# yukiteruono/pbsim3

Measured on AMD Instinct MI355X. Metric: simulated bases/sec, higher is better.
Workload: dtype u8

## Files before the change

pbsim3_amd/csrc/deflate.hip:

```cpp
#include <hip/hip_runtime.h>
#include <stdint.h>
#include <stdlib.h>

#include "kernels.h"

namespace pbsim {

namespace {

constexpr int kChunk = DF_CHUNK;
constexpr int kThreads = 256;
constexpr int kSeg = kChunk / kThreads;
constexpr int kSegDw = kSeg / 4;
constexpr int kInDw = kChunk / 4 + kChunk / 128;
constexpr int kOutBytes = 33024;
constexpr int kOutDw = kOutBytes / 4;
constexpr int kSyms = 288;
constexpr uint32_t kPoly = 0xEDB88320u;
constexpr int kHeadBits = 18 * 8;
constexpr int kPrefixBits = 3 + 5 + 5 + 4 + 19 * 3;

constexpr int kClLenTab[19] = {3, 5, 4, 4, 4, 5, 5, 5, 5, 5, 5, 5, 4, 5, 5, 5, 5, 3, 3};
constexpr int kClOrderTab[19] = {16, 17, 18, 0, 8, 7, 9, 6, 10, 5, 11, 4, 12, 3, 13, 2, 14, 1, 15};
constexpr uint64_t pack_cl_len() {
  uint64_t v = 0;
  for (int s = 0; s < 19; ++s) v |= (uint64_t)kClLenTab[s] << (3 * s);
  return v;
}
constexpr uint64_t kClLenPacked = pack_cl_len();
__device__ __forceinline__ uint32_t cl_len(uint32_t s) { return (uint32_t)(kClLenPacked >> (3 * s)) & 7u; }
constexpr unsigned __int128 pack_prefix() {
  unsigned __int128 v = 1u | (2u << 1) | ((unsigned __int128)15 << 13);
  for (int i = 0; i < 19; ++i) v |= (unsigned __int128)kClLenTab[kClOrderTab[i]] << (17 + 3 * i);
  return v;
}
constexpr uint64_t kPrefixLo = (uint64_t)pack_prefix();
constexpr uint32_t kPrefixHi = (uint32_t)(pack_prefix() >> 64);

__device__ __forceinline__ uint32_t rev_bits(uint32_t code, uint32_t len) { return __brev(code) >> (32 - len); }

__device__ __forceinline__ uint32_t cl_code(uint32_t s) {
  uint32_t c, l = cl_len(s);
  if (l == 3) c = s == 0 ? 0 : s - 16;
  else if (l == 4) c = s == 12 ? 9 : 4 + s;
  else c = s == 1 ? 20 : s <= 11 ? 16 + s : 15 + s;
  return rev_bits(c, l);
}

__device__ __forceinline__ uint32_t gf2_mul(uint32_t a, uint32_t b) {
  uint32_t p = 0;
#pragma unroll
  for (int i = 0; i < 32; ++i) {
    p ^= b & (0u - ((a >> (31 - i)) & 1u));
    b = (b >> 1) ^ (kPoly & (0u - (b & 1u)));
  }
  return p;
}

struct BitWriter {
  uint32_t *out;
  uint32_t word, nb;
  uint64_t acc;
  __device__ __forceinline__ void init(uint32_t *o, uint32_t bitpos) {
    out = o;
    word = bitpos >> 5;
    nb = bitpos & 31;
    acc = 0;
  }
  __device__ __forceinline__ void put(uint32_t v, uint32_t k) {
    acc |= (uint64_t)v << nb;
    nb += k;
    if (nb >= 32) {
      atomicOr(&out[word++], (uint32_t)acc);
      acc >>= 32;
      nb -= 32;
    }
  }
  __device__ __forceinline__ void put64(uint64_t v, uint32_t k) {
    if (k > 32) {
      put((uint32_t)v, 32);
      put((uint32_t)(v >> 32), k - 32);
    } else {
      put((uint32_t)v, k);
    }
  }
  __device__ __forceinline__ void flush() {
    if (nb) atomicOr(&out[word], (uint32_t)acc);
  }
};

__device__ __forceinline__ void length_symbol(uint32_t L, uint32_t *sym, uint32_t *eb, uint32_t *ev) {
  const uint32_t v = L - 3;
  if (v < 8) {
    *sym = 257 + v;
    *eb = 0;
    *ev = 0;
  } else if (L == 258) {
    *sym = 285;
    *eb = 0;
    *ev = 0;
  } else {
    const uint32_t e = (31 - __clz(v)) - 2;
    *sym = 261 + 4 * e + ((v >> e) & 3);
    *eb = e;
    *ev = v & ((1u << e) - 1);
  }
}

__device__ __forceinline__ uint32_t block_scan_excl(uint32_t v, uint32_t *s_wave, uint32_t *total) {
  const int lane = threadIdx.x & 63, wave = threadIdx.x >> 6;
  uint32_t inc = v;
#pragma unroll
  for (int d = 1; d < 64; d <<= 1) {
    const uint32_t o = __shfl_up(inc, d, 64);
    if (lane >= d) inc += o;
  }
  __syncthreads();
  if (lane == 63) s_wave[wave] = inc;
  __syncthreads();
  uint32_t base = 0, tot = 0;
#pragma unroll
  for (int w = 0; w < kThreads / 64; ++w) {
    const uint32_t x = s_wave[w];
    if (w < wave) base += x;
    tot += x;
  }
  *total = tot;
  return base + inc - v;
}

struct Mask128 {
  uint64_t lo, hi;
};
__device__ __forceinline__ Mask128 m_and(Mask128 a, Mask128 b) { return {a.lo & b.lo, a.hi & b.hi}; }
__device__ __forceinline__ Mask128 m_or(Mask128 a, Mask128 b) { return {a.lo | b.lo, a.hi | b.hi}; }
__device__ __forceinline__ Mask128 m_not(Mask128 a) { return {~a.lo, ~a.hi}; }
template <int K>
__device__ __forceinline__ Mask128 m_shl(Mask128 a) { return {a.lo << K, (a.hi << K) | (a.lo >> (64 - K))}; }
template <int K>
__device__ __forceinline__ Mask128 m_shr(Mask128 a) { return {(a.lo >> K) | (a.hi << (64 - K)), a.hi >> K}; }
__device__ __forceinline__ uint32_t m_nibble(Mask128 a, int j) {
  return (uint32_t)((j < 16 ? a.lo >> (4 * j) : a.hi >> (4 * j - 64)) & 15u);
}
__device__ __forceinline__ int m_first(Mask128 a) { return a.lo ? __builtin_ctzll(a.lo) : 64 + __builtin_ctzll(a.hi); }
__device__ __forceinline__ Mask128 m_clear(Mask128 a, int pos) {
  if (pos < 64) a.lo &= ~(1ull << pos);
  else a.hi &= ~(1ull << (pos - 64));
  return a;
}
__device__ __forceinline__ int m_run(Mask128 m, int pos) {
  uint64_t lo, hi;
  if (pos == 0) {
    lo = m.lo;
    hi = m.hi;
  } else if (pos < 64) {
    lo = (m.lo >> pos) | (m.hi << (64 - pos));
    hi = m.hi >> pos;
  } else {
    lo = m.hi >> (pos - 64);
    hi = 0;
  }
  if (~lo) return __builtin_ctzll(~lo);
  return ~hi ? 64 + __builtin_ctzll(~hi) : 128;
}

struct SegTokens {
  Mask128 lit;
  Mask128 start;
  Mask128 cover;
};

__device__ __forceinline__ SegTokens seg_tokens(const uint32_t (&seg)[kSegDw], int seg_n, uint32_t prev_dword,
                                                bool chunk_start) {
  uint64_t e[2] = {0, 0};
  uint32_t pw = prev_dword;
#pragma unroll
  for (int j = 0; j < kSegDw; ++j) {
    const uint32_t w = seg[j];
    const uint32_t d = w ^ ((w << 8) | (pw >> 24));
    const uint32_t z = ~(((d & 0x7F7F7F7Fu) + 0x7F7F7F7Fu) | d | 0x7F7F7F7Fu);
    const uint32_t nib = (((z >> 7) * 0x00204081u) >> 21) & 15u;
    e[j >> 4] |= (uint64_t)nib << (4 * (j & 15));
    pw = w;
  }
  Mask128 valid;
  valid.lo = seg_n >= 64 ? ~0ull : (1ull << seg_n) - 1;
  valid.hi = seg_n >= 128 ? ~0ull : seg_n > 64 ? (1ull << (seg_n - 64)) - 1 : 0ull;
  Mask128 eq = {e[0] & valid.lo, e[1] & valid.hi};
  if (chunk_start) eq.lo &= ~1ull;
  const Mask128 r3 = m_and(eq, m_and(m_shr<1>(eq), m_shr<2>(eq)));
  SegTokens t;
  t.cover = m_or(r3, m_or(m_shl<1>(r3), m_shl<2>(r3)));
  t.start = m_and(t.cover, m_not(m_shl<1>(t.cover)));
  t.lit = m_and(valid, m_not(t.cover));
  return t;
}

constexpr int kSampleChunks = DF_SAMPLE_CHUNKS;
constexpr int kHdrDw = DF_TABLE_HDR_DW;

struct DfTable {
  uint32_t code[kSyms];
  uint32_t hdr_end_bits;
  uint32_t pad[3];
  uint32_t hdr[kHdrDw];
};
static_assert(sizeof(DfTable) <= DF_TABLE_BYTES, "DF_TABLE_BYTES too small");

__device__ __forceinline__ void load_chunk(const uint8_t *__restrict__ text, int64_t n_bytes, int64_t chunk, uint32_t *s_in,
                                           uint32_t (&seg)[kSegDw], int *n_out, int *seg_n_out, uint32_t *prev_dw) {
  const int tid = threadIdx.x;
  const int64_t base = chunk * (int64_t)kChunk;
  const int n = (int)((n_bytes - base) < (int64_t)kChunk ? (n_bytes - base) : (int64_t)kChunk);
  const uint4 *src4 = reinterpret_cast<const uint4 *>(text + base);
  for (int q = tid; q < kChunk / 16; q += kThreads) {
    uint4 v = make_uint4(0, 0, 0, 0);
    if (q * 16 < n) v = src4[q];
    const int d = q * 4;
    uint32_t *dst = &s_in[d + (d >> 5)];
    dst[0] = v.x;
    dst[1] = v.y;
    dst[2] = v.z;
    dst[3] = v.w;
  }
  __syncthreads();
  const int beg = tid * kSeg;
  *n_out = n;
  *seg_n_out = n - beg < 0 ? 0 : (n - beg < kSeg ? n - beg : kSeg);
#pragma unroll
  for (int j = 0; j < kSegDw; ++j) seg[j] = s_in[tid * (kSegDw + 1) + j];
  *prev_dw = tid ? s_in[tid * (kSegDw + 1) - 2] : 0u;
  __syncthreads();
}

__global__ __launch_bounds__(kThreads) void k_deflate_hist(const uint8_t *__restrict__ text, int64_t n_bytes,
                                                            uint32_t *__restrict__ hist) {
  __shared__ uint32_t s_in[kInDw];
  __shared__ uint32_t s_hist[3 * kSyms + 64];
  const int tid = threadIdx.x, lane = tid & 63;
  for (int i = tid; i < 3 * kSyms + 64; i += kThreads) s_hist[i] = 0;
  uint32_t seg[kSegDw], prev_dw;
  int n, seg_n;
  load_chunk(text, n_bytes, blockIdx.x, s_in, seg, &n, &seg_n, &prev_dw);
  const SegTokens tk = seg_tokens(seg, seg_n, prev_dw, tid == 0);
  const uint32_t copy = (uint32_t)(lane % 3) * kSyms, dummy = 3 * kSyms + lane;
#pragma unroll
  for (int j = 0; j < kSegDw; ++j) {
    const uint32_t nl = m_nibble(tk.lit, j);
    if (nl == 0) continue;
    const uint32_t w = seg[j];
#pragma unroll
    for (int k = 0; k < 4; ++k) atomicAdd(&s_hist[((nl >> k) & 1u) ? copy + ((w >> (8 * k)) & 255u) : dummy], 1u);
  }
  Mask128 st = tk.start;
  while (st.lo | st.hi) {
    const int pos = m_first(st);
    st = m_clear(st, pos);
    uint32_t sy, eb, ev;
    length_symbol((uint32_t)m_run(tk.cover, pos), &sy, &eb, &ev);
    atomicAdd(&s_hist[copy + sy], 1u);
  }
  __syncthreads();
  for (int i = tid; i < 286; i += kThreads) {
    const uint32_t f = s_hist[i] + s_hist[kSyms + i] + s_hist[2 * kSyms + i] + (i == 256 ? 1u : 0u);
    if (f) atomicAdd(&hist[i], f);
  }
}

__global__ __launch_bounds__(kThreads) void k_deflate_build(const uint32_t *__restrict__ hist, DfTable *__restrict__ tbl) {
  __shared__ uint32_t s_freq[kSyms], s_sfreq[kSyms], s_w[kSyms], s_code[kSyms];
  __shared__ uint16_t s_sorted[kSyms], s_par[kSyms], s_leafpar[kSyms], s_dep[kSyms];
  __shared__ uint8_t s_len[kSyms];
  __shared__ uint32_t s_cnt[16], s_first[16];
  __shared__ uint32_t s_img[4 + kHdrDw];
  const int tid = threadIdx.x;
  constexpr int m = 286;
  for (int i = tid; i < kSyms; i += kThreads) {
    s_freq[i] = i < m ? hist[i] + 1u : 0u;
    s_code[i] = 0;
    s_len[i] = 0;
  }
  for (int i = tid; i < 4 + kHdrDw; i += kThreads) s_img[i] = 0;
  if (tid < 16) s_cnt[tid] = 0;
  __syncthreads();
  for (int i = tid; i < m; i += kThreads) {
    const uint32_t fi = s_freq[i];
    uint32_t rank = 0;
    for (int u = 0; u < m; ++u) {
      const uint32_t g = s_freq[u];
      rank += (g < fi) | ((g == fi) & (u < i));
    }
    s_sorted[rank] = (uint16_t)i;
    s_sfreq[rank] = fi;
  }
  __syncthreads();
  if (tid == 0) {
    int leaf = 0, root = 0;
    for (int nxt = 0; nxt < m - 1; ++nxt) {
      uint32_t tot = 0;
      for (int k = 0; k < 2; ++k) {
        const bool take_leaf = leaf < m && (root >= nxt || s_sfreq[leaf] <= s_w[root]);
        if (take_leaf) {
          tot += s_sfreq[leaf];
          s_leafpar[leaf] = (uint16_t)nxt;
          ++leaf;
        } else {
          tot += s_w[root];
          s_par[root] = (uint16_t)nxt;
          ++root;
        }
      }
      s_w[nxt] = tot;
    }
    s_dep[m - 2] = 0;
    for (int i = m - 3; i >= 0; --i) s_dep[i] = s_dep[s_par[i]] + 1;
    for (int i = 0; i < m; ++i) {
      int d = s_dep[s_leafpar[i]] + 1;
      if (d > 15) d = 15;
      s_cnt[d] += 1;
    }
    uint32_t total = 0;
    for (int l = 1; l <= 15; ++l) total += s_cnt[l] << (15 - l);
    while (total > (1u << 15)) {
      s_cnt[15] -= 1;
      for (int l = 14; l >= 1; --l)
        if (s_cnt[l]) {
// ... 52 lines not shown
  for (int i = tid; i < kHdrDw; i += kThreads) tbl->hdr[i] = s_img[4 + i];
}

struct DfCtl {
  uint32_t ticket;
  uint32_t error;
  int64_t total;
};
static_assert(sizeof(DfCtl) == DF_CTL_BYTES, "DF_CTL_BYTES");

constexpr uint64_t kStSize = 1ull << 32, kStPrefix = 2ull << 32;
__device__ __forceinline__ uint64_t st_word(uint32_t epoch, uint64_t flag, uint32_t v) { return ((uint64_t)epoch << 34) | flag | v; }

__device__ __forceinline__ uint32_t look_back(const uint64_t *status, int64_t c, uint32_t epoch, int lane, uint32_t *error) {
  uint32_t sum = 0;
  int64_t hi = c - 1;
  for (uint32_t spins = 0;; spins++) {
    if (spins > (1u << 24)) {
      if (lane == 0) atomicOr(error, 1u);
      return sum;
    }
    const int64_t i = hi - lane;
    uint64_t w = 0;
    if (i >= 0) w = __hip_atomic_load(&status[i], __ATOMIC_RELAXED, __HIP_MEMORY_SCOPE_AGENT);
    const bool mine = i >= 0 && (uint32_t)(w >> 34) == epoch && ((w >> 32) & 3u) != 0;
    const uint64_t ready = __ballot(mine || i < 0);
    const uint64_t pref = __ballot(mine && ((w >> 32) & 3u) == 2u);
    const int k = ~ready ? __builtin_ctzll(~ready) : 64;
    const uint64_t usable = k >= 64 ? ~0ull : ((1ull << k) - 1);
    const uint64_t stop = pref & usable;
    if (stop) {
      const int e = __builtin_ctzll(stop);
      uint32_t v = (lane <= e && i >= 0) ? (uint32_t)w : 0u;
#pragma unroll
      for (int d = 32; d >= 1; d >>= 1) v += __shfl_xor(v, d, 64);
      return sum + v;
    }
    if (k == 0) {
      __builtin_amdgcn_s_sleep(2);
      continue;
    }
    uint32_t v = (lane < k && i >= 0) ? (uint32_t)w : 0u;
#pragma unroll
    for (int d = 32; d >= 1; d >>= 1) v += __shfl_xor(v, d, 64);
    sum += v;
    hi -= k;
    if (hi < 0) return sum;
  }
}

typedef uint32_t u32x4 __attribute__((ext_vector_type(4)));
__device__ __forceinline__ void store_member(uint8_t *dst, const uint32_t *s_img, uint32_t bytes, int tid) {
  const uint32_t head = min((uint32_t)((16u - ((uintptr_t)dst & 15u)) & 15u), bytes);
  const uint8_t *s8 = reinterpret_cast<const uint8_t *>(s_img);
  if ((uint32_t)tid < head) dst[tid] = s8[tid];
  const uint32_t nvec = (bytes - head) >> 4;
  const uint32_t sh = head & 3u, dw0 = head >> 2;
  u32x4 *d4 = reinterpret_cast<u32x4 *>(dst + head);
  for (uint32_t v = tid; v < nvec; v += kThreads) {
    const uint32_t *p = s_img + dw0 + 4u * v;
    const uint32_t a = p[0], b = p[1], c = p[2], d = p[3], e = p[4];
    u32x4 o;
    o.x = __builtin_amdgcn_alignbyte(b, a, sh);
    o.y = __builtin_amdgcn_alignbyte(c, b, sh);
    o.z = __builtin_amdgcn_alignbyte(d, c, sh);
    o.w = __builtin_amdgcn_alignbyte(e, d, sh);
    __builtin_nontemporal_store(o, &d4[v]);
  }
  const uint32_t done = head + 16u * nvec;
  if ((uint32_t)tid < bytes - done) dst[done + tid] = s8[done + tid];
}

__global__ __launch_bounds__(kThreads) void k_deflate_chunks(const uint8_t *__restrict__ text, int64_t n_bytes,
                                                              uint8_t *__restrict__ dense, uint64_t *__restrict__ status,
                                                              DfCtl *__restrict__ ctl, uint32_t epoch,
                                                              const uint32_t *__restrict__ crc_table,
                                                              const uint32_t *__restrict__ pow128, uint32_t x8rem,
                                                              const DfTable *__restrict__ tbl,
                                                              unsigned long long *__restrict__ prof) {
  __shared__ uint32_t s_in[kInDw];
  static_assert(kOutDw <= kInDw, "the output image must fit the input image");
  uint32_t *const s_out = s_in;
  __shared__ uint32_t s_code[kSyms];
  uint32_t *const s_crc = s_in;
  __shared__ uint32_t s_wave[kThreads / 64];
  __shared__ uint32_t s_misc[4];

  const int tid = threadIdx.x, lane = tid & 63;
  unsigned long long t_prev = prof ? wall_clock64() : 0;
  int phase = 0;
  auto mark = [&]() {
    if (prof && tid == 0) {
      const unsigned long long t = wall_clock64();
      atomicAdd(&prof[phase], t - t_prev);
      t_prev = t;
    }
    ++phase;
  };
  for (int i = tid; i < kSyms; i += kThreads) s_code[i] = i < 286 ? tbl->code[i] : 0u;
  if (tid < 4) s_misc[tid] = tid == 0 ? atomicAdd(&ctl->ticket, 1u) : 0u;
  __syncthreads();
  const int64_t chunk = s_misc[0];
  const int64_t n_chunks = (n_bytes + kChunk - 1) / kChunk;
  uint32_t seg[kSegDw], prev_dw;
  int n, seg_n;
  load_chunk(text, n_bytes, chunk, s_in, seg, &n, &seg_n, &prev_dw);
  const int beg = tid * kSeg;
  mark();
  for (int i = tid; i < kInDw; i += kThreads) s_in[i] = (i < 1024) ? crc_table[i] : 0u;
  __syncthreads();
  const SegTokens tk = seg_tokens(seg, seg_n, prev_dw, tid == 0);

  uint32_t tok_bits = 0;
  {
    uint32_t c = tid == 0 ? 0xFFFFFFFFu : 0u;
    const int full = seg_n >> 2;
#pragma unroll
    for (int j = 0; j < kSegDw; ++j) {
      if (j < full) {
        const uint32_t x = c ^ seg[j];
        c = s_crc[768 + (x & 255u)] ^ s_crc[512 + ((x >> 8) & 255u)] ^ s_crc[256 + ((x >> 16) & 255u)] ^ s_crc[x >> 24];
      } else if (j == full) {
        for (int k = 0; k < (seg_n & 3); ++k) c = s_crc[(c ^ (seg[j] >> (8 * k))) & 255u] ^ (c >> 8);
      }
    }
    const int q = n >> 7, r = n & 127;
    if (seg_n == kSeg && tid < q) {
      c = gf2_mul(c, pow128[q - tid - 1]);
      if (r) c = gf2_mul(c, x8rem);
    }
    if (seg_n == 0) c = 0;
#pragma unroll
    for (int d = 32; d >= 1; d >>= 1) c ^= __shfl_xor(c, d, 64);
    if (lane == 0) atomicXor(&s_misc[3], c);
  }
  mark();
  {
#pragma unroll
    for (int j = 0; j < kSegDw; ++j) {
      const uint32_t nl = m_nibble(tk.lit, j);
      if (nl == 0) continue;
      const uint32_t w = seg[j];
#pragma unroll
      for (int k = 0; k < 4; ++k)
        tok_bits += s_code[((nl >> k) & 1u) ? (w >> (8 * k)) & 255u : 287u] >> 16;
    }
    Mask128 st = tk.start;
    while (st.lo | st.hi) {
      const int pos = m_first(st);
      st = m_clear(st, pos);
      uint32_t sy, eb, ev;
      length_symbol((uint32_t)m_run(tk.cover, pos), &sy, &eb, &ev);
      tok_bits += (s_code[sy] >> 16) + eb + 1;
    }
  }
  uint32_t tok_total;
  const uint32_t tok_off = block_scan_excl(tok_bits, s_wave, &tok_total);
  const uint32_t hdr_end = tbl->hdr_end_bits;
  const uint32_t eob_len = s_code[256] >> 16;
  const uint32_t payload_bits = hdr_end - kHeadBits + tok_total + eob_len;
  const uint32_t payload_bytes = (payload_bits + 7) >> 3;
  const bool huff = (18 + payload_bytes + 8 <= (uint32_t)kOutBytes) && (payload_bytes < (uint32_t)n + 5);
  const uint32_t crc = s_misc[3] ^ 0xFFFFFFFFu;
  const uint32_t member = huff ? 18 + payload_bytes + 8 : 18 + 5 + (uint32_t)n + 8;
  if (tid == 0)
    __hip_atomic_store(&status[chunk], st_word(epoch, chunk == 0 ? kStPrefix : kStSize, member), __ATOMIC_RELAXED, __HIP_MEMORY_SCOPE_AGENT);
  mark();

  if (huff) {
    __syncthreads();
    for (int i = tid; i < 1024; i += kThreads) s_in[i] = 0;
    __syncthreads();
    if (tid < kHdrDw) s_out[4 + tid] = tbl->hdr[tid];
    if (tid == 0) {
      s_out[0] = 0x04088b1fu;
      s_out[1] = 0;
      s_out[2] = 0x0006ff00u;
      s_out[3] = 0x00024342u;
    }
    __syncthreads();
    if (tid == 0) atomicOr(&s_out[4], member - 1);
    mark();
    {
      BitWriter bw;
      bw.init(s_out, hdr_end + tok_off);
#pragma unroll
      for (int j = 0; j < kSegDw; ++j) {
        const uint32_t nl = m_nibble(tk.lit, j), ns = m_nibble(tk.start, j);
        if ((nl | ns) == 0) continue;
        const uint32_t w = seg[j];
        uint32_t c[4];
#pragma unroll
        for (int k = 0; k < 4; ++k) c[k] = s_code[((nl >> k) & 1u) ? (w >> (8 * k)) & 255u : 287u];
        uint32_t mv = 0, ml = 0, ks = 4;
        if (ns) {
          ks = (uint32_t)__builtin_ctz(ns);
          uint32_t sy, eb, ev;
          length_symbol((uint32_t)m_run(tk.cover, 4 * j + (int)ks), &sy, &eb, &ev);
          const uint32_t cm = s_code[sy];
          mv = (cm & 0xFFFFu) | (ev << (cm >> 16));
          ml = (cm >> 16) + eb + 1;
        }
        bw.put(ks == 0 ? mv : 0u, ks == 0 ? ml : 0u);
        {
          const uint32_t l0 = c[0] >> 16;
          bw.put((c[0] & 0xFFFFu) | ((c[1] & 0xFFFFu) << l0), l0 + (c[1] >> 16));
        }
        const bool mid = ks == 1 || ks == 2;
        bw.put(mid ? mv : 0u, mid ? ml : 0u);
        {
          const uint32_t l2 = c[2] >> 16;
          bw.put((c[2] & 0xFFFFu) | ((c[3] & 0xFFFFu) << l2), l2 + (c[3] >> 16));
        }
        bw.put(ks == 3 ? mv : 0u, ks == 3 ? ml : 0u);
      }
      bw.flush();
    }
    mark();
    if (tid == 0) {
      BitWriter bw;
      bw.init(s_out, hdr_end + tok_total);
      bw.put(s_code[256] & 0xFFFFu, eob_len);
      bw.flush();
      bw.init(s_out, (18 + payload_bytes) * 8);
      bw.put(crc, 32);
      bw.put((uint32_t)n, 32);
      bw.flush();
    }
    if (tid < 64 && chunk > 0) {
      const uint32_t excl = look_back(status, chunk, epoch, tid, &ctl->error);
      if (tid == 0) {
        s_misc[1] = excl;
        __hip_atomic_store(&status[chunk], st_word(epoch, kStPrefix, excl + member), __ATOMIC_RELAXED, __HIP_MEMORY_SCOPE_AGENT);
      }
    }
    __syncthreads();
    mark();
    const uint32_t off = s_misc[1];
    store_member(dense + off, s_out, member, tid);
    if (tid == 0 && chunk == n_chunks - 1) ctl->total = (int64_t)off + member;
    mark();
  } else {
    if (tid < 64 && chunk > 0) {
      const uint32_t excl = look_back(status, chunk, epoch, tid, &ctl->error);
      if (tid == 0) {
        s_misc[1] = excl;
        __hip_atomic_store(&status[chunk], st_word(epoch, kStPrefix, excl + member), __ATOMIC_RELAXED, __HIP_MEMORY_SCOPE_AGENT);
      }
    }
    __syncthreads();
    uint8_t *slot = dense + s_misc[1];
    if (tid == 0 && chunk == n_chunks - 1) ctl->total = (int64_t)s_misc[1] + member;
    if (tid == 0) {
      const uint8_t head[23] = {0x1f, 0x8b, 8,   4,   0,   0,
                                0,    0,    0,   0xff, 6,  0,
                                'B',  'C',  2,   0,   (uint8_t)((member - 1) & 255), (uint8_t)((member - 1) >> 8),
                                1,    (uint8_t)(n & 255), (uint8_t)(n >> 8), (uint8_t)(~n & 255), (uint8_t)((~n >> 8) & 255)};
      for (int i = 0; i < 23; ++i) slot[i] = head[i];
      uint8_t *t = slot + 23 + n;
      for (int i = 0; i < 4; ++i) t[i] = (uint8_t)(crc >> (8 * i));
      for (int i = 0; i < 4; ++i) t[4 + i] = (uint8_t)((uint32_t)n >> (8 * i));
    }
#pragma unroll
    for (int j = 0; j < kSegDw; ++j)
#pragma unroll
      for (int k = 0; k < 4; ++k)
        if (4 * j + k < seg_n) slot[23 + beg + 4 * j + k] = (uint8_t)(seg[j] >> (8 * k));
  }
}

uint32_t host_gf2_mul(uint32_t a, uint32_t b) {
  uint32_t p = 0;
  for (int i = 0; i < 32; ++i) {
    if (a & (0x80000000u >> i)) p ^= b;
    b = (b >> 1) ^ ((b & 1u) ? kPoly : 0u);
  }
  return p;
}

uint32_t host_xpow8(uint64_t nbytes) {
  uint32_t r = 0x80000000u, b = 0x00800000u;
  while (nbytes) {
    if (nbytes & 1) r = host_gf2_mul(r, b);
    b = host_gf2_mul(b, b);
    nbytes >>= 1;
  }
  return r;
}

}

void deflate_host_tables(uint32_t *crc_table, uint32_t *pow128) {
  for (uint32_t i = 0; i < 256; ++i) {
    uint32_t c = i;
    for (int k = 0; k < 8; ++k) c = (c >> 1) ^ ((c & 1u) ? kPoly : 0u);
    crc_table[i] = c;
  }
  for (int t = 1; t < 4; ++t)
    for (uint32_t i = 0; i < 256; ++i) {
      const uint32_t c = crc_table[(t - 1) * 256 + i];
      crc_table[t * 256 + i] = (c >> 8) ^ crc_table[c & 255u];
    }
  const uint32_t step = host_xpow8(128);
  uint32_t v = 0x80000000u;
  for (int k = 0; k < 256; ++k) {
    pow128[k] = v;
    v = host_gf2_mul(v, step);
  }
}

void launch_deflate_table(const uint8_t *text, int64_t n_bytes, uint32_t *hist, void *table, hipStream_t s) {
  if (n_bytes <= 0) return;
  const int64_t nch = (n_bytes + DF_CHUNK - 1) / DF_CHUNK;
  const int64_t ns = nch < kSampleChunks ? nch : kSampleChunks;
  const int64_t sample_bytes = ns * (int64_t)DF_CHUNK < n_bytes ? ns * (int64_t)DF_CHUNK : n_bytes;
  (void)hipMemsetAsync(hist, 0, 288 * sizeof(uint32_t), s);
  hipLaunchKernelGGL(k_deflate_hist, dim3((unsigned)ns), dim3(kThreads), 0, s, text, sample_bytes, hist);
  hipLaunchKernelGGL(k_deflate_build, dim3(1), dim3(kThreads), 0, s, (const uint32_t *)hist, reinterpret_cast<DfTable *>(table));
}

void launch_deflate(const uint8_t *text, int64_t n_bytes, uint64_t *status, void *ctl, uint32_t epoch, uint8_t *dense,
                    const uint32_t *d_crc_table, const uint32_t *d_pow128, const void *table, hipStream_t s,
                    unsigned long long *d_prof, hipEvent_t ev_begin, hipEvent_t ev_chunks_done) {
  if (n_bytes <= 0) return;
  const int64_t nch = (n_bytes + DF_CHUNK - 1) / DF_CHUNK;
  const uint32_t x8rem = host_xpow8((uint64_t)(n_bytes % DF_CHUNK) & 127u);
  (void)hipMemsetAsync(ctl, 0, DF_CTL_BYTES, s);
  if (ev_begin) (void)hipEventRecord(ev_begin, s);
  hipLaunchKernelGGL(k_deflate_chunks, dim3((unsigned)nch), dim3(kThreads), 0, s, text, n_bytes, dense, status,
                     reinterpret_cast<DfCtl *>(ctl), epoch & 0x3fffffffu, d_crc_table, d_pow128, x8rem,
                     reinterpret_cast<const DfTable *>(table), d_prof);
  if (ev_chunks_done) (void)hipEventRecord(ev_chunks_done, s);
}

}
```

pbsim3_amd/csrc/deflate_host.cpp:

```cpp
#include <hip/hip_runtime.h>
#include <limits.h>
#include <math.h>
#include <stdio.h>
#include <stdlib.h>
#include <string.h>

#include <algorithm>
#include <chrono>
#include <functional>
#include <memory>
#include <string>
#include <thread>
#include <vector>

#include "ctx.h"
#include "engine_internal.h"
#include "unit_io.h"

extern "C" {

extern "C++" {
namespace {

int ensure_deflate_tables(pbsim_ctx *c) {
// ... 129 lines not shown
  bool used[kDfBuffers] = {false};
  int64_t *h_total = reinterpret_cast<int64_t *>(sl.h_df_total.p);
  auto launch = [&](int64_t j) -> int {
    return df_launch_piece(c, sl, g, d_text, n, j, used[(int)(j % nbuf)], place == nullptr, d_prof);
  };
  for (int64_t j = sl.pre_count; j < std::min<int64_t>(ahead, n_pieces); j++)
    if (!launch(j)) return PBSIM_FAILED;
  const char *prev_ptr = nullptr;
  int64_t prev_bytes = 0;
  int prev_buf = 0;
  for (int64_t k = 0; k < n_pieces; k++) {
    const int b = (int)(k % nbuf);
    const double t0 = now();
    HIP_OK(hipEventSynchronize(sl.ev_df[b]));
    t_kernel += now() - t0;
    const int64_t total = h_total[2 * b + 1];
    if ((uint64_t)h_total[2 * b] >> 32) return fail("deflate: a workgroup's look-back gave up waiting for its predecessors");
    out_bytes += total;
    {
      float ms = 0;
      if (hipEventElapsedTime(&ms, sl.ev_k0[b], sl.ev_k1[b]) == hipSuccess) {
        std::lock_guard<std::mutex> lk(c->prof_mu);
        c->prof_deflate_ms += ms;
        c->prof_deflate_launches++;
        c->prof_deflate_in += g.len(k, n);
        c->prof_deflate_out += total;
      }
    }
    char *dst = place ? (*place)(total) : (char *)sl.h_df_out[b].p;
    if (!dst) return fail("deflate: no room for a compressed piece");
    HIP_OK(hipStreamWaitEvent(sl.copy_stream, sl.ev_df[b], 0));
    if (trace) {
      hipEvent_t e0 = nullptr, e1 = nullptr;
      HIP_OK(hipEventCreate(&e0));
      HIP_OK(hipEventCreate(&e1));
      tev.emplace_back(e0, e1);
      HIP_OK(hipEventRecord(e0, sl.copy_stream));
    }
    HIP_OK(hipMemcpyAsync(dst, sl.d_df_dense[b].p, (size_t)total, hipMemcpyDeviceToHost, sl.copy_stream));
    if (trace) HIP_OK(hipEventRecord(tev.back().second, sl.copy_stream));
    HIP_OK(hipEventRecord(sl.ev_cp[b], sl.copy_stream));
    used[b] = true;
    if (prev_bytes) {
      const double t1 = now();
      HIP_OK(hipEventSynchronize(sl.ev_cp[prev_buf]));
      const double t2 = now();
      if (!consume(prev_ptr, prev_bytes)) return PBSIM_FAILED;
      t_copy += t2 - t1;
      t_consume += now() - t2;
    }
    prev_ptr = dst;
    prev_bytes = total;
    prev_buf = b;
    if (k + ahead < n_pieces && !launch(k + ahead)) return PBSIM_FAILED;
  }
  if (prev_bytes) {
    const double t1 = now();
    HIP_OK(hipEventSynchronize(sl.ev_cp[prev_buf]));
    const double t2 = now();
    if (!consume(prev_ptr, prev_bytes)) return PBSIM_FAILED;
    t_copy += t2 - t1;
    t_consume += now() - t2;
  }
  if (trace) {
    double t_link = 0, t_span = 0;
    float ms = 0;
    for (auto &e : tev) {
      if (hipEventElapsedTime(&ms, e.first, e.second) == hipSuccess) t_link += ms;
    }
    if (!tev.empty() && hipEventElapsedTime(&ms, tev.front().first, tev.back().second) == hipSuccess) t_span = ms;
    for (auto &e : tev) {
      (void)hipEventDestroy(e.first);
      (void)hipEventDestroy(e.second);
    }
    fprintf(stderr,
            "[deflate] %.1f MB -> %.1f MB in %.1f ms: waited %.1f ms for kernels, %.1f ms for copies, %.1f ms in the consumer; copies: "
            "%.1f ms on the engine within a span of %.1f ms (%.1f GB/s while copying)\n",
            n / 1e6, out_bytes / 1e6, now() - t_begin, t_kernel, t_copy, t_consume, t_link, t_span, t_link > 0 ? out_bytes / t_link / 1e6 : 0.0);
  }
  if (d_prof) {
    unsigned long long t[16];
    HIP_OK(hipMemcpy(t, d_prof, 128, hipMemcpyDeviceToHost));
    const double nch = (double)((n + DF_CHUNK - 1) / DF_CHUNK);
    static const char *names[7] = {"stage", "crc", "sizes+scan", "header", "tokens", "trailer", "store"};
    fprintf(stderr, "[deflate prof] %.0f chunks; us per chunk (lane 0):", nch);
    for (int i = 0; i < 7; ++i) fprintf(stderr, " %s %.1f", names[i], t[i] / nch / 100);
    fprintf(stderr, "\n");
  }
  return PBSIM_SUCCEEDED;
}

int deflate_to_host(pbsim_ctx *c, DfLane &sl, const uint8_t *d_text, int64_t n, char *host_dst, int64_t cap,
                    int64_t *out_bytes) {
  int64_t written = 0;
  const int ok = deflate_stream(c, sl, d_text, n, [&](const char *z, int64_t k) {
    if (written + k > cap) return fail("deflate: output buffer too small");
    memcpy(host_dst + written, z, (size_t)k);
    written += k;
    return PBSIM_SUCCEEDED;
  });
  *out_bytes = written;
  return ok;
}

}
}

extern "C++" int pbsim::deflate_pieces(pbsim_ctx *c, DfLane &lane, const uint8_t *d_text, int64_t n,
                                       const std::function<int(const char *, int64_t)> &consume,
                                       const std::function<char *(int64_t)> *place) {
  return deflate_stream(c, lane, d_text, n, consume, place);
}
extern "C++" int pbsim::ensure_deflate_ready(pbsim_ctx *c) {
  for (auto &lane : c->df_streams)
    for (hipStream_t &st : lane)
      if (!st) HIP_OK(hipStreamCreateWithFlags(&st, hipStreamNonBlocking));
  return ensure_deflate_tables(c);
}
extern "C++" int pbsim::ensure_crc_tables(pbsim_ctx *c) { return ensure_deflate_tables(c); }
extern "C++" int pbsim::deflate_prelaunch(pbsim_ctx *c, Slot &sl, bool want_read, bool want_maf) {
  const pbsim_batch_info &bi = sl.b_info;
  if (want_read && bi.read_text_bytes > 0 && !df_begin(c, sl.df[0], sl.d_read_text.as<uint8_t>(), bi.read_text_bytes, true, sl.stream))
    return PBSIM_FAILED;
  if (want_maf && bi.maf_text_bytes > 0 && !df_begin(c, sl.df[1], sl.d_maf_text.as<uint8_t>(), bi.maf_text_bytes, true, sl.stream))
    return PBSIM_FAILED;
  return PBSIM_SUCCEEDED;
}

int pbsim_set_deflate(pbsim_ctx *c, int on) {
  if (!c) return fail("bad argument");
  c->deflate = on & 3;
  c->deflate_parallel = (on & 4) != 0;
  return PBSIM_SUCCEEDED;
}

int64_t pbsim_deflate_bound(int64_t n) {
  if (n <= 0) return 0;
  return n + ((n + DF_CHUNK - 1) / DF_CHUNK) * 31;
}

int pbsim_batch_fetch_deflated(pbsim_ctx *c, char *read_gz, int64_t read_cap, char *maf_gz, int64_t maf_cap,
                               int64_t *read_gz_bytes, int64_t *maf_gz_bytes) {
  if (!c || !c->s().b_finalized) return fail("pbsim_batch_fetch_deflated: no finalized batch");
  NEED_DEVICE(c);
  HIP_OK(hipSetDevice(c->device));
  int64_t nr = 0, nm = 0;
  if (read_gz && !deflate_to_host(c, c->s().df[0], c->s().d_read_text.as<uint8_t>(), c->s().b_info.read_text_bytes, read_gz,
                                  read_cap, &nr))
    return PBSIM_FAILED;
  if (maf_gz && !deflate_to_host(c, c->s().df[0], c->s().d_maf_text.as<uint8_t>(), c->s().b_info.maf_text_bytes, maf_gz,
                                 maf_cap, &nm))
    return PBSIM_FAILED;
  if (read_gz_bytes) *read_gz_bytes = nr;
  if (maf_gz_bytes) *maf_gz_bytes = nm;
  return PBSIM_SUCCEEDED;
}

int pbsim_deflate_buffer(pbsim_ctx *c, const void *src, int64_t n, void *dst, int64_t cap, int64_t *out_bytes) {
  if (!c || !out_bytes || n < 0 || (n > 0 && (!src || !dst))) return fail("pbsim_deflate_buffer: bad argument");
  NEED_DEVICE(c);
  HIP_OK(hipSetDevice(c->device));
  *out_bytes = 0;
  if (n == 0) return PBSIM_SUCCEEDED;
  Slot &sl = c->slots[0];
  DevBuf d_in;
  HIP_OK(d_in.ensure((size_t)n + 16));
  HIP_OK(hipMemcpyAsync(d_in.p, src, (size_t)n, hipMemcpyHostToDevice, sl.stream));
  HIP_OK(hipStreamSynchronize(sl.stream));
  return deflate_to_host(c, sl.df[0], d_in.as<uint8_t>(), n, (char *)dst, cap, out_bytes);
// ... 68 lines not shown
```

Before: 56.38 billion.

## Make deflate kernel persistent with prefetch of next chunk and resident CRC table

Turns k_deflate_chunks into a persistent kernel: the grid is capped at the number of resident workgroups, and each workgroup loops over chunks taken from the ticket counter. The next chunk's global load is issued before the current member is stored, so the fetch overlaps the store. The CRC table, header dwords and code table are now loaded once per workgroup into a dedicated shared array instead of once per chunk. The zeroing of the output image is limited to the member size, and the bit writer uses branchless puts. The cost is 4 KB more LDS per workgroup, which may lower occupancy, and more register pressure from keeping the prefetched quads live.

Measured after the change: 56.38 billion (median of 3 runs). No clear change (+0.0%).

```diff
diff --git a/pbsim3_amd/csrc/deflate.hip b/pbsim3_amd/csrc/deflate.hip
--- a/pbsim3_amd/csrc/deflate.hip
+++ b/pbsim3_amd/csrc/deflate.hip
@@ -1,6 +1,9 @@
 #include <hip/hip_runtime.h>
 #include <stdint.h>
 #include <stdlib.h>
+
+#include <algorithm>
+#include <atomic>
 
 #include "kernels.h"
 
@@ -75,6 +78,15 @@
       acc >>= 32;
       nb -= 32;
     }
+  }
+  __device__ __forceinline__ void put_always(uint32_t v, uint32_t k) {
+    acc |= (uint64_t)v << nb;
+    nb += k;
+    atomicOr(&out[word], (uint32_t)acc);
+    const bool full = nb >= 32;
+    word += full ? 1u : 0u;
+    acc = full ? acc >> 32 : acc;
+    nb &= 31u;
   }
   __device__ __forceinline__ void put64(uint64_t v, uint32_t k) {
     if (k > 32) {
@@ -107,8 +119,8 @@
   }
 }
 
-__device__ __forceinline__ uint32_t block_scan_excl(uint32_t v, uint32_t *s_wave, uint32_t *total) {
-  const int lane = threadIdx.x & 63, wave = threadIdx.x >> 6;
+__device__ __forceinline__ uint32_t block_scan_excl(uint32_t v, uint32_t *s_wave, uint32_t *total, int tid) {
+  const int lane = tid & 63, wave = tid >> 6;
   uint32_t inc = v;
 #pragma unroll
   for (int d = 1; d < 64; d <<= 1) {
@@ -207,30 +219,40 @@
 };
 static_assert(sizeof(DfTable) <= DF_TABLE_BYTES, "DF_TABLE_BYTES too small");
 
-__device__ __forceinline__ void load_chunk(const uint8_t *__restrict__ text, int64_t n_bytes, int64_t chunk, uint32_t *s_in,
-                                           uint32_t (&seg)[kSegDw], int *n_out, int *seg_n_out, uint32_t *prev_dw) {
-  const int tid = threadIdx.x;
-  const int64_t base = chunk * (int64_t)kChunk;
-  const int n = (int)((n_bytes - base) < (int64_t)kChunk ? (n_bytes - base) : (int64_t)kChunk);
-  const uint4 *src4 = reinterpret_cast<const uint4 *>(text + base);
-  for (int q = tid; q < kChunk / 16; q += kThreads) {
-    uint4 v = make_uint4(0, 0, 0, 0);
-    if (q * 16 < n) v = src4[q];
-    const int d = q * 4;
+constexpr int kQuads = kChunk / 16 / kThreads;
+__device__ __forceinline__ int chunk_bytes(int64_t n_bytes, int64_t chunk) {
+  const int64_t left = n_bytes - chunk * (int64_t)kChunk;
+  return (int)(left < 0 ? 0 : left < (int64_t)kChunk ? left : (int64_t)kChunk);
+}
+__device__ __forceinline__ void chunk_fetch(const uint8_t *__restrict__ text, int64_t n_bytes, int64_t chunk, uint4 (&quad)[kQuads], int tid) {
+  const int n = chunk_bytes(n_bytes, chunk);
+  const uint4 *src4 = reinterpret_cast<const uint4 *>(text + chunk * (int64_t)kChunk);
+#pragma unroll
+  for (int i = 0; i < kQuads; ++i) {
+    const int q = tid + i * kThreads;
+    quad[i] = make_uint4(0, 0, 0, 0);
+    if (q * 16 < n) quad[i] = src4[q];
+  }
+}
+__device__ __forceinline__ void chunk_land(const uint4 (&quad)[kQuads], int64_t n_bytes, int64_t chunk, uint32_t *s_in,
+                                           uint32_t (&seg)[kSegDw], int *n_out, int *seg_n_out, uint32_t *prev_dw, int tid) {
+#pragma unroll
+  for (int i = 0; i < kQuads; ++i) {
+    const int d = (tid + i * kThreads) * 4;
     uint32_t *dst = &s_in[d + (d >> 5)];
-    dst[0] = v.x;
-    dst[1] = v.y;
-    dst[2] = v.z;
-    dst[3] = v.w;
-  }
-  __syncthreads();
+    dst[0] = quad[i].x;
+    dst[1] = quad[i].y;
+    dst[2] = quad[i].z;
+    dst[3] = quad[i].w;
+  }
+  __syncthreads();
+  const int n = chunk_bytes(n_bytes, chunk);
   const int beg = tid * kSeg;
   *n_out = n;
   *seg_n_out = n - beg < 0 ? 0 : (n - beg < kSeg ? n - beg : kSeg);
 #pragma unroll
   for (int j = 0; j < kSegDw; ++j) seg[j] = s_in[tid * (kSegDw + 1) + j];
   *prev_dw = tid ? s_in[tid * (kSegDw + 1) - 2] : 0u;
-  __syncthreads();
 }
 
 __global__ __launch_bounds__(kThreads) void k_deflate_hist(const uint8_t *__restrict__ text, int64_t n_bytes,
@@ -241,7 +263,9 @@
   for (int i = tid; i < 3 * kSyms + 64; i += kThreads) s_hist[i] = 0;
   uint32_t seg[kSegDw], prev_dw;
   int n, seg_n;
-  load_chunk(text, n_bytes, blockIdx.x, s_in, seg, &n, &seg_n, &prev_dw);
+  uint4 quad[kQuads];
+  chunk_fetch(text, n_bytes, blockIdx.x, quad, tid);
+  chunk_land(quad, n_bytes, blockIdx.x, s_in, seg, &n, &seg_n, &prev_dw, tid);
   const SegTokens tk = seg_tokens(seg, seg_n, prev_dw, tid == 0);
   const uint32_t copy = (uint32_t)(lane % 3) * kSyms, dummy = 3 * kSyms + lane;
 #pragma unroll
@@ -460,190 +484,205 @@
   static_assert(kOutDw <= kInDw, "the output image must fit the input image");
   uint32_t *const s_out = s_in;
   __shared__ uint32_t s_code[kSyms];
-  uint32_t *const s_crc = s_in;
+  __shared__ uint32_t s_crc[1024];
   __shared__ uint32_t s_wave[kThreads / 64];
   __shared__ uint32_t s_misc[4];
 
-  const int tid = threadIdx.x, lane = tid & 63;
+  const int tid0 = threadIdx.x;
   unsigned long long t_prev = prof ? wall_clock64() : 0;
-  int phase = 0;
+  int phase = 7;
   auto mark = [&]() {
-    if (prof && tid == 0) {
+    if (prof && tid0 == 0) {
       const unsigned long long t = wall_clock64();
       atomicAdd(&prof[phase], t - t_prev);
       t_prev = t;
     }
     ++phase;
   };
-  for (int i = tid; i < kSyms; i += kThreads) s_code[i] = i < 286 ? tbl->code[i] : 0u;
-  if (tid < 4) s_misc[tid] = tid == 0 ? atomicAdd(&ctl->ticket, 1u) : 0u;
-  __syncthreads();
-  const int64_t chunk = s_misc[0];
   const int64_t n_chunks = (n_bytes + kChunk - 1) / kChunk;
-  uint32_t seg[kSegDw], prev_dw;
-  int n, seg_n;
-  load_chunk(text, n_bytes, chunk, s_in, seg, &n, &seg_n, &prev_dw);
-  const int beg = tid * kSeg;
+  for (int i = tid0; i < kSyms; i += kThreads) s_code[i] = i < 286 ? tbl->code[i] : 0u;
+  for (int i = tid0; i < 1024; i += kThreads) s_crc[i] = crc_table[i];
+  static_assert(kHdrDw <= kThreads, "one header dword per thread");
+  const uint32_t my_hdr = tid0 < kHdrDw ? tbl->hdr[tid0] : 0u;
+  const uint32_t hdr_end = tbl->hdr_end_bits;
+  if (tid0 < 4) s_misc[tid0] = tid0 == 0 ? atomicAdd(&ctl->ticket, 1u) : 0u;
+  __syncthreads();
+  int64_t chunk = s_misc[0];
+  const uint32_t eob = s_code[256], eob_len = eob >> 16;
+  uint4 quad[kQuads];
+  chunk_fetch(text, n_bytes, chunk, quad, tid0);
   mark();
-  for (int i = tid; i < kInDw; i += kThreads) s_in[i] = (i < 1024) ? crc_table[i] : 0u;
-  __syncthreads();
-  const SegTokens tk = seg_tokens(seg, seg_n, prev_dw, tid == 0);
-
-  uint32_t tok_bits = 0;
-  {
-    uint32_t c = tid == 0 ? 0xFFFFFFFFu : 0u;
-    const int full = seg_n >> 2;
-#pragma unroll
-    for (int j = 0; j < kSegDw; ++j) {
-      if (j < full) {
-        const uint32_t x = c ^ seg[j];
-        c = s_crc[768 + (x & 255u)] ^ s_crc[512 + ((x >> 8) & 255u)] ^ s_crc[256 + ((x >> 16) & 255u)] ^ s_crc[x >> 24];
-      } else if (j == full) {
-        for (int k = 0; k < (seg_n & 3); ++k) c = s_crc[(c ^ (seg[j] >> (8 * k))) & 255u] ^ (c >> 8);
-      }
-    }
-    const int q = n >> 7, r = n & 127;
-    if (seg_n == kSeg && tid < q) {
-      c = gf2_mul(c, pow128[q - tid - 1]);
-      if (r) c = gf2_mul(c, x8rem);
-    }
-    if (seg_n == 0) c = 0;
-#pragma unroll
-    for (int d = 32; d >= 1; d >>= 1) c ^= __shfl_xor(c, d, 64);
-    if (lane == 0) atomicXor(&s_misc[3], c);
-  }
-  mark();
-  {
-#pragma unroll
-    for (int j = 0; j < kSegDw; ++j) {
-      const uint32_t nl = m_nibble(tk.lit, j);
-      if (nl == 0) continue;
-      const uint32_t w = seg[j];
-#pragma unroll
-      for (int k = 0; k < 4; ++k)
-        tok_bits += s_code[((nl >> k) & 1u) ? (w >> (8 * k)) & 255u : 287u] >> 16;
-    }
-    Mask128 st = tk.start;
-    while (st.lo | st.hi) {
-      const int pos = m_first(st);
-      st = m_clear(st, pos);
-      uint32_t sy, eb, ev;
-      length_symbol((uint32_t)m_run(tk.cover, pos), &sy, &eb, &ev);
-      tok_bits += (s_code[sy] >> 16) + eb + 1;
-    }
-  }
-  uint32_t tok_total;
-  const uint32_t tok_off = block_scan_excl(tok_bits, s_wave, &tok_total);
-  const uint32_t hdr_end = tbl->hdr_end_bits;
-  const uint32_t eob_len = s_code[256] >> 16;
-  const uint32_t payload_bits = hdr_end - kHeadBits + tok_total + eob_len;
-  const uint32_t payload_bytes = (payload_bits + 7) >> 3;
-  const bool huff = (18 + payload_bytes + 8 <= (uint32_t)kOutBytes) && (payload_bytes < (uint32_t)n + 5);
-  const uint32_t crc = s_misc[3] ^ 0xFFFFFFFFu;
-  const uint32_t member = huff ? 18 + payload_bytes + 8 : 18 + 5 + (uint32_t)n + 8;
-  if (tid == 0)
-    __hip_atomic_store(&status[chunk], st_word(epoch, chunk == 0 ? kStPrefix : kStSize, member), __ATOMIC_RELAXED, __HIP_MEMORY_SCOPE_AGENT);
-  mark();
-
-  if (huff) {
-    __syncthreads();
-    for (int i = tid; i < 1024; i += kThreads) s_in[i] = 0;
-    __syncthreads();
-    if (tid < kHdrDw) s_out[4 + tid] = tbl->hdr[tid];
-    if (tid == 0) {
-      s_out[0] = 0x04088b1fu;
-      s_out[1] = 0;
-      s_out[2] = 0x0006ff00u;
-      s_out[3] = 0x00024342u;
-    }
-    __syncthreads();
-    if (tid == 0) atomicOr(&s_out[4], member - 1);
+
+  while (chunk < n_chunks) {
+    phase = 0;
+    int tid = tid0;
+    __asm__ volatile("" : "+v"(tid));
+    __asm__ volatile("" : "+s"(x8rem));
+    const int lane = tid & 63;
+    uint32_t seg[kSegDw], prev_dw;
+    int n, seg_n;
+    chunk_land(quad, n_bytes, chunk, s_in, seg, &n, &seg_n, &prev_dw, tid);
+    const int beg = tid * kSeg;
+    mark();
+    SegTokens tk = seg_tokens(seg, seg_n, prev_dw, tid == 0);
+
+    uint32_t tok_bits = 0;
+    {
+      uint32_t c = tid == 0 ? 0xFFFFFFFFu : 0u;
+      const int full = seg_n >> 2;
+#pragma unroll
+      for (int j = 0; j < kSegDw; ++j) {
+        if (j < full) {
+          const uint32_t x = c ^ seg[j];
+          c = s_crc[768 + (x & 255u)] ^ s_crc[512 + ((x >> 8) & 255u)] ^ s_crc[256 + ((x >> 16) & 255u)] ^ s_crc[x >> 24];
+        } else if (j == full) {
+          for (int k = 0; k < (seg_n & 3); ++k) c = s_crc[(c ^ (seg[j] >> (8 * k))) & 255u] ^ (c >> 8);
+        }
+      }
+      const int q = n >> 7, r = n & 127;
+      if (seg_n == kSeg && tid < q) {
+        c = gf2_mul(c, pow128[q - tid - 1]);
+        if (r) c = gf2_mul(c, x8rem);
+      }
+      if (seg_n == 0) c = 0;
+#pragma unroll
+      for (int d = 32; d >= 1; d >>= 1) c ^= __shfl_xor(c, d, 64);
+      if (lane == 0) atomicXor(&s_misc[3], c);
+    }
     mark();
     {
-      BitWriter bw;
-      bw.init(s_out, hdr_end + tok_off);
 #pragma unroll
       for (int j = 0; j < kSegDw; ++j) {
-        const uint32_t nl = m_nibble(tk.lit, j), ns = m_nibble(tk.start, j);
-        if ((nl | ns) == 0) continue;
+        const uint32_t nl = m_nibble(tk.lit, j);
+        if (nl == 0) continue;
         const uint32_t w = seg[j];
-        uint32_t c[4];
-#pragma unroll
-        for (int k = 0; k < 4; ++k) c[k] = s_code[((nl >> k) & 1u) ? (w >> (8 * k)) & 255u : 287u];
-        uint32_t mv = 0, ml = 0, ks = 4;
-        if (ns) {
-          ks = (uint32_t)__builtin_ctz(ns);
-          uint32_t sy, eb, ev;
-          length_symbol((uint32_t)m_run(tk.cover, 4 * j + (int)ks), &sy, &eb, &ev);
-          const uint32_t cm = s_code[sy];
-          mv = (cm & 0xFFFFu) | (ev << (cm >> 16));
-          ml = (cm >> 16) + eb + 1;
+#pragma unroll
+        for (int k = 0; k < 4; ++k)
+          tok_bits += s_code[((nl >> k) & 1u) ? (w >> (8 * k)) & 255u : 287u] >> 16;
+      }
+      Mask128 st = tk.start;
+      while (st.lo | st.hi) {
+        const int pos = m_first(st);
+        st = m_clear(st, pos);
+        uint32_t sy, eb, ev;
+        length_symbol((uint32_t)m_run(tk.cover, pos), &sy, &eb, &ev);
+        tok_bits += (s_code[sy] >> 16) + eb + 1;
+      }
+    }
+    uint32_t tok_total;
+    const uint32_t tok_off = block_scan_excl(tok_bits, s_wave, &tok_total, tid);
+    const uint32_t payload_bits = hdr_end - kHeadBits + tok_total + eob_len;
+    const uint32_t payload_bytes = (payload_bits + 7) >> 3;
+    const bool huff = (18 + payload_bytes + 8 <= (uint32_t)kOutBytes) && (payload_bytes < (uint32_t)n + 5);
+    const uint32_t member = huff ? 18 + payload_bytes + 8 : 18 + 5 + (uint32_t)n + 8;
+    uint32_t crc = 0;
+    if (tid == 0) {
+      __hip_atomic_store(&status[chunk], st_word(epoch, chunk == 0 ? kStPrefix : kStSize, member), __ATOMIC_RELAXED, __HIP_MEMORY_SCOPE_AGENT);
+      crc = s_misc[3] ^ 0xFFFFFFFFu;
+      s_misc[3] = 0;
+    }
+    mark();
+    int64_t next_chunk;
+
+    if (huff) {
+      const uint32_t img_dw = (member + 3) >> 2;
+      for (uint32_t i = 4 + kHdrDw + tid; i < img_dw; i += kThreads) s_out[i] = 0;
+      if (tid < kHdrDw) s_out[4 + tid] = my_hdr | (tid == 0 ? member - 1 : 0u);
+      if (tid >= 128 && tid < 132) s_out[tid - 128] = tid == 128 ? 0x04088b1fu : tid == 129 ? 0u : tid == 130 ? 0x0006ff00u : 0x00024342u;
+      __syncthreads();
+      mark();
+      {
+        __asm__ volatile("" : "+v"(tk.lit.lo), "+v"(tk.lit.hi), "+v"(tk.start.lo), "+v"(tk.start.hi));
+        BitWriter bw;
+        bw.init(s_out, hdr_end + tok_off);
+#pragma unroll
+        for (int j = 0; j < kSegDw; ++j) {
+          const uint32_t nl = m_nibble(tk.lit, j), ns = m_nibble(tk.start, j);
+          if ((nl | ns) == 0) continue;
+          const uint32_t w = seg[j];
+          uint32_t c[4];
+#pragma unroll
+          for (int k = 0; k < 4; ++k) c[k] = s_code[((nl >> k) & 1u) ? (w >> (8 * k)) & 255u : 287u];
+          uint32_t mv = 0, ml = 0, ks = 4;
+          if (ns) {
+            ks = (uint32_t)__builtin_ctz(ns);
+            uint32_t sy, eb, ev;
+            length_symbol((uint32_t)m_run(tk.cover, 4 * j + (int)ks), &sy, &eb, &ev);
+            const uint32_t cm = s_code[sy];
+            mv = (cm & 0xFFFFu) | (ev << (cm >> 16));
+            ml = (cm >> 16) + eb + 1;
+          }
+          const uint32_t l0 = c[0] >> 16, l2 = c[2] >> 16;
+          const uint32_t v01 = (c[0] & 0xFFFFu) | ((c[1] & 0xFFFFu) << l0), n01 = l0 + (c[1] >> 16);
+          const uint32_t v23 = (c[2] & 0xFFFFu) | ((c[3] & 0xFFFFu) << l2), n23 = l2 + (c[3] >> 16);
+          const bool mid = ks == 1 || ks == 2;
+          bw.put_always(ks == 0 ? mv : v01, ks == 0 ? ml : n01);
+          bw.put_always(mid ? mv : v23, mid ? ml : n23);
+          bw.put_always(ks == 3 ? mv : 0u, ks == 3 ? ml : 0u);
         }
-        bw.put(ks == 0 ? mv : 0u, ks == 0 ? ml : 0u);
-        {
-          const uint32_t l0 = c[0] >> 16;
-          bw.put((c[0] & 0xFFFFu) | ((c[1] & 0xFFFFu) << l0), l0 + (c[1] >> 16));
+        bw.flush();
+      }
+      mark();
+      if (tid == 0) {
+        BitWriter bw;
+        bw.init(s_out, hdr_end + tok_total);
+        bw.put(eob & 0xFFFFu, eob_len);
+        bw.flush();
+        bw.init(s_out, (18 + payload_bytes) * 8);
+        bw.put(crc, 32);
+        bw.put((uint32_t)n, 32);
+        bw.flush();
+      }
+      if (tid < 64) {
+        const uint32_t excl = chunk > 0 ? look_back(status, chunk, epoch, tid, &ctl->error) : 0u;
+        if (tid == 0) {
+          s_misc[1] = excl;
+          if (chunk > 0)
+            __hip_atomic_store(&status[chunk], st_word(epoch, kStPrefix, excl + member), __ATOMIC_RELAXED, __HIP_MEMORY_SCOPE_AGENT);
+          s_misc[0] = atomicAdd(&ctl->ticket, 1u);
         }
-        const bool mid = ks == 1 || ks == 2;
-        bw.put(mid ? mv : 0u, mid ? ml : 0u);
-        {
-          const uint32_t l2 = c[2] >> 16;
-          bw.put((c[2] & 0xFFFFu) | ((c[3] & 0xFFFFu) << l2), l2 + (c[3] >> 16));
+      }
+      __syncthreads();
+      mark();
+      next_chunk = s_misc[0];
+      chunk_fetch(text, n_bytes, next_chunk, quad, tid);
+      const uint32_t off = s_misc[1];
+      store_member(dense + off, s_out, member, tid);
+      if (tid == 0 && chunk == n_chunks - 1) ctl->total = (int64_t)off + member;
+      mark();
+    } else {
+      if (tid < 64) {
+        const uint32_t excl = chunk > 0 ? look_back(status, chunk, epoch, tid, &ctl->error) : 0u;
+        if (tid == 0) {
+          s_misc[1] = excl;
+          if (chunk > 0)
+            __hip_atomic_store(&status[chunk], st_word(epoch, kStPrefix, excl + member), __ATOMIC_RELAXED, __HIP_MEMORY_SCOPE_AGENT);
+          s_misc[0] = atomicAdd(&ctl->ticket, 1u);
         }
-        bw.put(ks == 3 ? mv : 0u, ks == 3 ? ml : 0u);
-      }
-      bw.flush();
-    }
-    mark();
-    if (tid == 0) {
-      BitWriter bw;
-      bw.init(s_out, hdr_end + tok_total);
-      bw.put(s_code[256] & 0xFFFFu, eob_len);
-      bw.flush();
-      bw.init(s_out, (18 + payload_bytes) * 8);
-      bw.put(crc, 32);
-      bw.put((uint32_t)n, 32);
-      bw.flush();
-    }
-    if (tid < 64 && chunk > 0) {
-      const uint32_t excl = look_back(status, chunk, epoch, tid, &ctl->error);
+      }
+      __syncthreads();
+      next_chunk = s_misc[0];
+      uint8_t *slot = dense + s_misc[1];
+      if (tid == 0 && chunk == n_chunks - 1) ctl->total = (int64_t)s_misc[1] + member;
       if (tid == 0) {
-        s_misc[1] = excl;
-        __hip_atomic_store(&status[chunk], st_word(epoch, kStPrefix, excl + member), __ATOMIC_RELAXED, __HIP_MEMORY_SCOPE_AGENT);
-      }
+        const uint8_t head[23] = {0x1f, 0x8b, 8,   4,   0,   0,
+                                  0,    0,    0,   0xff, 6,  0,
+                                  'B',  'C',  2,   0,   (uint8_t)((member - 1) & 255), (uint8_t)((member - 1) >> 8),
+                                  1,    (uint8_t)(n & 255), (uint8_t)(n >> 8), (uint8_t)(~n & 255), (uint8_t)((~n >> 8) & 255)};
+        for (int i = 0; i < 23; ++i) slot[i] = head[i];
+        uint8_t *t = slot + 23 + n;
+        for (int i = 0; i < 4; ++i) t[i] = (uint8_t)(crc >> (8 * i));
+        for (int i = 0; i < 4; ++i) t[4 + i] = (uint8_t)((uint32_t)n >> (8 * i));
+      }
+#pragma unroll
+      for (int j = 0; j < kSegDw; ++j)
+#pragma unroll
+        for (int k = 0; k < 4; ++k)
+          if (4 * j + k < seg_n) slot[23 + beg + 4 * j + k] = (uint8_t)(seg[j] >> (8 * k));
+      chunk_fetch(text, n_bytes, next_chunk, quad, tid);
     }
     __syncthreads();
-    mark();
-    const uint32_t off = s_misc[1];
-    store_member(dense + off, s_out, member, tid);
-    if (tid == 0 && chunk == n_chunks - 1) ctl->total = (int64_t)off + member;
-    mark();
-  } else {
-    if (tid < 64 && chunk > 0) {
-      const uint32_t excl = look_back(status, chunk, epoch, tid, &ctl->error);
-      if (tid == 0) {
-        s_misc[1] = excl;
-        __hip_atomic_store(&status[chunk], st_word(epoch, kStPrefix, excl + member), __ATOMIC_RELAXED, __HIP_MEMORY_SCOPE_AGENT);
-      }
-    }
-    __syncthreads();
-    uint8_t *slot = dense + s_misc[1];
-    if (tid == 0 && chunk == n_chunks - 1) ctl->total = (int64_t)s_misc[1] + member;
-    if (tid == 0) {
-      const uint8_t head[23] = {0x1f, 0x8b, 8,   4,   0,   0,
-                                0,    0,    0,   0xff, 6,  0,
-                                'B',  'C',  2,   0,   (uint8_t)((member - 1) & 255), (uint8_t)((member - 1) >> 8),
-                                1,    (uint8_t)(n & 255), (uint8_t)(n >> 8), (uint8_t)(~n & 255), (uint8_t)((~n >> 8) & 255)};
-      for (int i = 0; i < 23; ++i) slot[i] = head[i];
-      uint8_t *t = slot + 23 + n;
-      for (int i = 0; i < 4; ++i) t[i] = (uint8_t)(crc >> (8 * i));
-      for (int i = 0; i < 4; ++i) t[4 + i] = (uint8_t)((uint32_t)n >> (8 * i));
-    }
-#pragma unroll
-    for (int j = 0; j < kSegDw; ++j)
-#pragma unroll
-      for (int k = 0; k < 4; ++k)
-        if (4 * j + k < seg_n) slot[23 + beg + 4 * j + k] = (uint8_t)(seg[j] >> (8 * k));
+    chunk = next_chunk;
   }
 }
 
@@ -685,6 +724,21 @@
     pow128[k] = v;
     v = host_gf2_mul(v, step);
   }
+}
+
+static int deflate_resident_workgroups() {
+  constexpr int kMaxDev = 64;
+  static std::atomic<int> cached[kMaxDev];
+  int dev = 0;
+  if (hipGetDevice(&dev) != hipSuccess || dev < 0 || dev >= kMaxDev) dev = 0;
+  int g = cached[dev].load(std::memory_order_relaxed);
+  if (g > 0) return g;
+  int cus = 0, per_cu = 0;
+  if (hipDeviceGetAttribute(&cus, hipDeviceAttributeMultiprocessorCount, dev) != hipSuccess || cus <= 0) cus = 1;
+  if (hipOccupancyMaxActiveBlocksPerMultiprocessor(&per_cu, k_deflate_chunks, kThreads, 0) != hipSuccess || per_cu <= 0) per_cu = 1;
+  g = cus * per_cu;
+  cached[dev].store(g, std::memory_order_relaxed);
+  return g;
 }
 
 void launch_deflate_table(const uint8_t *text, int64_t n_bytes, uint32_t *hist, void *table, hipStream_t s) {
@@ -705,7 +759,8 @@
   const uint32_t x8rem = host_xpow8((uint64_t)(n_bytes % DF_CHUNK) & 127u);
   (void)hipMemsetAsync(ctl, 0, DF_CTL_BYTES, s);
   if (ev_begin) (void)hipEventRecord(ev_begin, s);
-  hipLaunchKernelGGL(k_deflate_chunks, dim3((unsigned)nch), dim3(kThreads), 0, s, text, n_bytes, dense, status,
+  const int64_t grid = std::min<int64_t>(nch, deflate_resident_workgroups());
+  hipLaunchKernelGGL(k_deflate_chunks, dim3((unsigned)grid), dim3(kThreads), 0, s, text, n_bytes, dense, status,
                      reinterpret_cast<DfCtl *>(ctl), epoch & 0x3fffffffu, d_crc_table, d_pow128, x8rem,
                      reinterpret_cast<const DfTable *>(table), d_prof);
   if (ev_chunks_done) (void)hipEventRecord(ev_chunks_done, s);
diff --git a/pbsim3_amd/csrc/deflate_host.cpp b/pbsim3_amd/csrc/deflate_host.cpp
--- a/pbsim3_amd/csrc/deflate_host.cpp
+++ b/pbsim3_amd/csrc/deflate_host.cpp
@@ -235,9 +235,9 @@
     unsigned long long t[16];
     HIP_OK(hipMemcpy(t, d_prof, 128, hipMemcpyDeviceToHost));
     const double nch = (double)((n + DF_CHUNK - 1) / DF_CHUNK);
-    static const char *names[7] = {"stage", "crc", "sizes+scan", "header", "tokens", "trailer", "store"};
+    static const char *names[8] = {"land", "crc", "sizes+scan", "zero+header", "tokens", "trailer", "store", "setup"};
     fprintf(stderr, "[deflate prof] %.0f chunks; us per chunk (lane 0):", nch);
-    for (int i = 0; i < 7; ++i) fprintf(stderr, " %s %.1f", names[i], t[i] / nch / 100);
+    for (int i = 0; i < 8; ++i) fprintf(stderr, " %s %.1f", names[i], t[i] / nch / 100);
     fprintf(stderr, "\n");
   }
   return PBSIM_SUCCEEDED;
```
